# victorramirez952/tomography_3d_reconstructor

Measured on AMD Instinct MI355X. Metric: Mvoxels/s (SDF+MC) on 1024^3 ellipsoid stack; achieved HBM GB/s vs peak, higher is better.
Workload: dtype f64

## Files before the change

tomography_3d_reconstructor_amd/csrc/mesh.hip:

```cpp
#include <cstring>
#include <cstdlib>
#include "tomo_common.h"
#include <rocprim/rocprim.hpp>

__global__ __launch_bounds__(256) void vertex_finalize_kernel(float *__restrict__ vpos, int64_t nv, int shift,
                                                              const double *__restrict__ cum, int64_t ncum,
                                                              const double *__restrict__ adj, int64_t nadj, float mm_y,
                                                              float mm_x)
{
    int64_t i = (int64_t)blockIdx.x * blockDim.x + threadIdx.x;
    if (i >= nv) return;
    float *p = vpos + 3 * i;
    float z = p[0], y = p[1], x = p[2];
    if (shift) { z -= 1.0f; y -= 1.0f; x -= 1.0f; }
    if (nadj > 0) {
        if (z < 0.0f) z = 0.0f;
        else if ((double)z >= (double)(ncum - 1)) z = (float)cum[ncum - 1];
        else {
            int64_t lo = (int64_t)floorf(z);
            float frac = z - (float)lo;
            int64_t k = lo < nadj - 1 ? lo : nadj - 1;
            z = (float)(cum[lo] + (double)frac * adj[k]);
        }
    }
    p[0] = z; p[1] = y * mm_y; p[2] = x * mm_x;
}

TOMO_API int tomo_vertex_finalize(float *vpos, int64_t nv, int shift, const double *cum, int64_t ncum, const double *adj,
                                  int64_t nadj, float mm_y, float mm_x, void *stream)
{
    if (nv < 0 || (nv > 0 && !vpos) || (nadj > 0 && (!cum || !adj || ncum != nadj + 1))) return TOMO_E_ARG;
    if (nv == 0) return TOMO_OK;
    int64_t blocks = ceil_div64(nv, 256);
    if (blocks > 0x7fffffff) return TOMO_E_SIZE;
    hipLaunchKernelGGL(vertex_finalize_kernel, dim3((unsigned)blocks), dim3(256), 0, (hipStream_t)stream, vpos, nv, shift,
                       cum, ncum, adj, nadj, mm_y, mm_x);
    return tomo_status();
}

__device__ static inline u32 fkey32(float f)
{
    u32 u = __float_as_uint(f);
    return (u & 0x80000000u) ? ~u : (u | 0x80000000u);
}

__global__ __launch_bounds__(256) void uq_init_kernel(const float *__restrict__ vpos, int64_t nv, u32 *__restrict__ kx,
                                                      u32 *__restrict__ idx)
{
    int64_t i = (int64_t)blockIdx.x * blockDim.x + threadIdx.x;
    if (i >= nv) return;
    kx[i] = fkey32(vpos[3 * i + 2]);
    idx[i] = (u32)i;
}

__global__ __launch_bounds__(256) void uq_gather_kernel(const float *__restrict__ vpos, int64_t nv,
                                                        const u32 *__restrict__ idx, u64 *__restrict__ kzy)
{
    int64_t i = (int64_t)blockIdx.x * blockDim.x + threadIdx.x;
    if (i >= nv) return;
    const float *p = vpos + 3 * (int64_t)idx[i];
    kzy[i] = ((u64)fkey32(p[0]) << 32) | (u64)fkey32(p[1]);
}

__global__ __launch_bounds__(256) void uq_heads_kernel(const float *__restrict__ vpos, int64_t nv,
                                                       const u32 *__restrict__ idx, u32 *__restrict__ head)
{
    int64_t i = (int64_t)blockIdx.x * blockDim.x + threadIdx.x;
    if (i >= nv) return;
    u32 h = 1;
    if (i > 0) {
        const float *a = vpos + 3 * (int64_t)idx[i], *b = vpos + 3 * (int64_t)idx[i - 1];
        h = (a[0] != b[0] || a[1] != b[1] || a[2] != b[2]) ? 1u : 0u;
    }
    head[i] = h;
}

__global__ __launch_bounds__(256) void uq_scatter_kernel(const float *__restrict__ vpos, int64_t nv,
                                                         const u32 *__restrict__ idx, const u32 *__restrict__ head,
                                                         const u32 *__restrict__ hscan, float *__restrict__ uniq,
                                                         int32_t *__restrict__ rank, u64 *__restrict__ totals)
{
    int64_t i = (int64_t)blockIdx.x * blockDim.x + threadIdx.x;
    if (i >= nv) return;
    u32 u = hscan[i] - 1u;
    u32 src = idx[i];
    rank[src] = (int32_t)u;
    if (head[i]) {
        const float *p = vpos + 3 * (int64_t)src;
        float *q = uniq + 3 * (int64_t)u;
        q[0] = p[0]; q[1] = p[1]; q[2] = p[2];
    }
    if (i == nv - 1) totals[0] = (u64)hscan[i];
}

struct UqLayout {
    size_t kx_a, kx_b, idx_a, idx_b, idx_c, kzy_a, kzy_b, head, hscan, temp, temp_bytes, total;
};

static inline size_t align_up(size_t x, size_t a) { return (x + a - 1) / a * a; }

static UqLayout uq_layout(int64_t nv)
{
    UqLayout L;
    size_t n = (size_t)(nv > 0 ? nv : 1), off = 0;
    auto take = [&](size_t bytes) { size_t o = off; off = align_up(off + bytes, 256); return o; };
    L.kx_a = take(n * 4); L.kx_b = take(n * 4);
    L.idx_a = take(n * 4); L.idx_b = take(n * 4); L.idx_c = take(n * 4);
    L.kzy_a = take(n * 8); L.kzy_b = take(n * 8);
    L.head = take(n * 4); L.hscan = take(n * 4);
    size_t t1 = 0, t2 = 0, t3 = 0;
    (void)rocprim::radix_sort_pairs(nullptr, t1, (u32 *)nullptr, (u32 *)nullptr, (u32 *)nullptr, (u32 *)nullptr, n, 0, 32,
                              (hipStream_t)0);
    (void)rocprim::radix_sort_pairs(nullptr, t2, (u64 *)nullptr, (u64 *)nullptr, (u32 *)nullptr, (u32 *)nullptr, n, 0, 64,
                              (hipStream_t)0);
    (void)rocprim::inclusive_scan(nullptr, t3, (u32 *)nullptr, (u32 *)nullptr, n, rocprim::plus<u32>(), (hipStream_t)0);
    L.temp_bytes = t1 > t2 ? t1 : t2;
    if (t3 > L.temp_bytes) L.temp_bytes = t3;
    L.temp = take(L.temp_bytes + 256);
    L.total = off;
    return L;
}

TOMO_API int64_t tomo_mesh_unique_workspace_bytes(int64_t nv) { return (int64_t)uq_layout(nv).total; }

TOMO_API int tomo_mesh_unique(const float *vpos, int64_t nv, float *uniq, int32_t *rank, unsigned long long *totals,
                              void *workspace, int64_t workspace_bytes, void *stream)
{
    if (!vpos || !uniq || !rank || !totals || !workspace || nv <= 0) return TOMO_E_ARG;
    if (nv >= 0x7fffffffll) return TOMO_E_SIZE;
    UqLayout L = uq_layout(nv);
    if ((size_t)workspace_bytes < L.total) return TOMO_E_WORKSPACE;
    char *ws = (char *)workspace;
    u32 *kx_a = (u32 *)(ws + L.kx_a), *kx_b = (u32 *)(ws + L.kx_b);
    u32 *idx_a = (u32 *)(ws + L.idx_a), *idx_b = (u32 *)(ws + L.idx_b), *idx_c = (u32 *)(ws + L.idx_c);
    u64 *kzy_a = (u64 *)(ws + L.kzy_a), *kzy_b = (u64 *)(ws + L.kzy_b);
    u32 *head = (u32 *)(ws + L.head), *hscan = (u32 *)(ws + L.hscan);
    void *temp = ws + L.temp;
    size_t tb = L.temp_bytes;
    hipStream_t s = (hipStream_t)stream;
    unsigned blocks = (unsigned)ceil_div64(nv, 256);
    hipLaunchKernelGGL(uq_init_kernel, dim3(blocks), dim3(256), 0, s, vpos, nv, kx_a, idx_a);
    if (rocprim::radix_sort_pairs(temp, tb, kx_a, kx_b, idx_a, idx_b, (size_t)nv, 0, 32, s) != hipSuccess) return TOMO_E_LAUNCH;
    hipLaunchKernelGGL(uq_gather_kernel, dim3(blocks), dim3(256), 0, s, vpos, nv, (const u32 *)idx_b, kzy_a);
    tb = L.temp_bytes;
    if (rocprim::radix_sort_pairs(temp, tb, kzy_a, kzy_b, idx_b, idx_c, (size_t)nv, 0, 64, s) != hipSuccess) return TOMO_E_LAUNCH;
    hipLaunchKernelGGL(uq_heads_kernel, dim3(blocks), dim3(256), 0, s, vpos, nv, (const u32 *)idx_c, head);
    tb = L.temp_bytes;
    if (rocprim::inclusive_scan(temp, tb, head, hscan, (size_t)nv, rocprim::plus<u32>(), s) != hipSuccess) return TOMO_E_LAUNCH;
    hipLaunchKernelGGL(uq_scatter_kernel, dim3(blocks), dim3(256), 0, s, vpos, nv, (const u32 *)idx_c, (const u32 *)head,
                       (const u32 *)hscan, uniq, rank, (u64 *)totals);
    return tomo_status();
}

#define UQ_MAX_SLABS 65536

typedef rocprim::segmented_radix_sort_config<8, rocprim::kernel_config<512, 8>, rocprim::WarpSortConfig<32, 4, 256, 0x7fffffff, 32, 4, 256>, true>
    UqSegCfg;

struct UqOrder {
    const u32 *idx, *alt, *off;
    __device__ u32 at(u32 i) const
    {
        if (off != nullptr && i >= off[1] && i < off[3]) return alt[i];
        return idx[i];
    }
};

__device__ static inline bool rec_less(const float4 &a, const float4 &b)
{
    return a.x < b.x || (a.x == b.x && (a.y < b.y || (a.y == b.y && a.z < b.z)));
}

__global__ __launch_bounds__(256) void uq3_merge_kernel(const float4 *__restrict__ vrec, const u32 *__restrict__ off,
                                                        const u32 *__restrict__ idx, u32 *__restrict__ alt)
{
    const u32 o1 = off[1], o2 = off[2], o3 = off[3];
    const u32 na = o2 - o1, nb = o3 - o2;
    for (u32 t = blockIdx.x * blockDim.x + threadIdx.x; t < na + nb; t += gridDim.x * blockDim.x) {
        const bool inA = t < na;
        const u32 src = idx[inA ? o1 + t : o2 + (t - na)];
        const float4 k = vrec[src];
        const u32 base = inA ? o2 : o1;
        u32 lo = 0, hi = inA ? nb : na;
        while (lo < hi) {
            const u32 mid = lo + ((hi - lo) >> 1);
            const float4 m = vrec[idx[base + mid]];
            const bool less = rec_less(m, k);
            const bool equal = m.x == k.x && m.y == k.y && m.z == k.z;
            if (less || (!inA && equal)) lo = mid + 1; else hi = mid;
        }
        alt[o1 + (inA ? t : t - na) + lo] = src;
    }
}

__global__ __launch_bounds__(256) void uq3_rank_kernel(const float4 *__restrict__ vrec, int64_t cap_v, const UqOrder ord,
                                                       float *__restrict__ uniq, int32_t *__restrict__ table,
                                                       u64 *__restrict__ tot, const float z_top)
{
    const int64_t i = (int64_t)blockIdx.x * blockDim.x + threadIdx.x;
    bool viol = false;
    const u64 nv = tot[1];
    const bool live = tot[3] == 0 && i < cap_v && (u64)i < nv;
    float4 a = make_float4(0.f, 0.f, 0.f, 0.f);
    if (live) {
        u32 sa = ord.at((u32)i);
        if ((u64)sa >= nv) { sa = 0; viol = true; }
        a = vrec[sa];
    }
    float4 b;
    b.x = __shfl_up(a.x, 1, 64); b.y = __shfl_up(a.y, 1, 64); b.z = __shfl_up(a.z, 1, 64);
    if (live) {
        if ((threadIdx.x & 63) == 0 && i > 0) {
            u32 sb = ord.at((u32)i - 1u);
            if ((u64)sb >= nv) { sb = 0; viol = true; }
            b = vrec[sb];
        }
        if (i > 0) viol = viol || !rec_less(b, a);
        typedef float f3u __attribute__((ext_vector_type(3), aligned(4)));
        *(f3u *)(uniq + 3 * i) = (f3u){a.x, a.y, a.z};
        table[__float_as_uint(a.w)] = (int32_t)i;
    }
    const u64 n = (u64)__popcll(__ballot(viol));
    if ((threadIdx.x & 63) == 0 && n) atomicAdd((unsigned long long *)&tot[4], (unsigned long long)n);
    const u64 nt = (u64)__popcll(__ballot(live && a.x == z_top));
    if ((threadIdx.x & 63) == 0 && nt) atomicAdd((unsigned long long *)&tot[7], (unsigned long long)nt);
}

struct Uq3Layout { size_t keys_alt, idx_alt, idx_merge, temp, temp_bytes, total; };

static Uq3Layout uq3_layout(int64_t cap_v, int64_t nseg)
{
    Uq3Layout L;
    size_t n = (size_t)(cap_v > 0 ? cap_v : 1), off = 0;
    auto take = [&](size_t bytes) { size_t o = off; off = align_up(off + bytes, 256); return o; };
    L.keys_alt = take(n * 4); L.idx_alt = take(n * 4); L.idx_merge = take(n * 4);
    size_t t = 0;
    (void)rocprim::segmented_radix_sort_pairs<UqSegCfg>(nullptr, t, (u32 *)nullptr, (u32 *)nullptr, (u32 *)nullptr, (u32 *)nullptr,
                                                        (unsigned)n, (unsigned)(nseg > 0 ? nseg : 1), (const u32 *)nullptr,
                                                        (const u32 *)nullptr, 0, 32, (hipStream_t)0);
    L.temp_bytes = t;
    L.temp = take(t + 256);
    L.total = off;
    return L;
}

TOMO_API int64_t tomo_mc3_sort_workspace_bytes(int64_t cap_v, int64_t nseg) { return (int64_t)uq3_layout(cap_v, nseg).total; }

TOMO_API int tomo_mc3_sort_rank_top(const float *vrec, uint32_t *keys, uint32_t *idx, int64_t cap_v, int Nz, int Ny,
                                    const uint32_t *slice_tab, unsigned long long *tot, float *uniq, int32_t *table, void *workspace,
                                    int64_t workspace_bytes, float z_top, void *stream)
{
    if (!vrec || !keys || !idx || !slice_tab || !tot || !uniq || !table || !workspace || cap_v <= 0 || Nz < 1 || Ny < 1) return TOMO_E_ARG;
    if (cap_v >= 0x7fffffffll || Nz > UQ_MAX_SLABS) return TOMO_E_SIZE;
    const int64_t nseg = (int64_t)(TOMO_SORT_NB(Ny) + 1) * Nz;
    if (nseg >= 0x7fffffffll) return TOMO_E_SIZE;
    Uq3Layout L = uq3_layout(cap_v, nseg);
    if ((size_t)workspace_bytes < L.total) return TOMO_E_WORKSPACE;
    char *ws = (char *)workspace;
    u32 *keys_alt = (u32 *)(ws + L.keys_alt), *idx_alt = (u32 *)(ws + L.idx_alt), *idx_merge = (u32 *)(ws + L.idx_merge);
    const u32 *offsets = slice_tab + 2 * ((int64_t)Nz + 1);
    const u32 *merge3 = offsets + nseg + 1;
    hipStream_t s = (hipStream_t)stream;
    size_t tb = L.temp_bytes;
    if (rocprim::segmented_radix_sort_pairs<UqSegCfg>(ws + L.temp, tb, keys, keys_alt, idx, idx_alt, (unsigned)cap_v, (unsigned)nseg,
                                                      offsets, offsets + 1, 0, 32, s) != hipSuccess)
        return TOMO_E_LAUNCH;
    UqOrder order{(const u32 *)idx_alt, nullptr, nullptr};
    if (Nz >= 2) {
        hipLaunchKernelGGL(uq3_merge_kernel, dim3(256), dim3(256), 0, s, (const float4 *)vrec, merge3 - 1, (const u32 *)idx_alt, idx_merge);
        order.alt = idx_merge;
        order.off = merge3 - 1;
    }
    hipLaunchKernelGGL(uq3_rank_kernel, dim3((unsigned)ceil_div64(cap_v, 256)), dim3(256), 0, s, (const float4 *)vrec, cap_v, order,
                       uniq, table, (u64 *)tot, z_top);
    return tomo_status();
}

#define SR_THREADS 256
#define SR_E 8
#define SR_CAP 4096
#define SR_HALF 2048
#define SR_PAD(i) ((i) + ((i) >> 3))
#define SR_WORDS(cap) ((cap) + ((cap) >> 3))
#define SR_RUN (64 * SR_E)

template <int M>
__device__ static inline u32 sr_lane_xor(u32 x, const int lane)
{
    const int v = (int)x;
    if (M == 1) return (u32)__builtin_amdgcn_update_dpp(v, v, 0xB1 , 0xf, 0xf, false);
    if (M == 2) return (u32)__builtin_amdgcn_update_dpp(v, v, 0x4E , 0xf, 0xf, false);
    if (M == 8) return (u32)__builtin_amdgcn_update_dpp(v, v, 0x128 , 0xf, 0xf, false);
    if (M == 4) {
        const int up = __builtin_amdgcn_update_dpp(v, v, 0x104 , 0xf, 0xf, false);
        const int dn = __builtin_amdgcn_update_dpp(v, v, 0x114 , 0xf, 0xf, false);
        return (u32)((lane & 4) ? dn : up);
    }
    return (u32)__shfl_xor(v, M, 64);
}
template <int M>
__device__ static inline u64 sr_shfl_xor(u64 v, const int lane)
{
    return ((u64)sr_lane_xor<M>((u32)(v >> 32), lane) << 32) | sr_lane_xor<M>((u32)v, lane);
}

template <int K, int J>
__device__ static inline void sr_stage(u64 (&v)[SR_E], const int lane)
{
    if (J >= SR_E) {
        constexpr int M = J / SR_E;
        const bool keep_min = ((((lane * SR_E) & K) == 0) == ((lane & M) == 0));
#pragma unroll
        for (int r = 0; r < SR_E; r++) {
            const u64 o = sr_shfl_xor<(M > 0 ? M : 1)>(v[r], lane);
            v[r] = (keep_min == (o < v[r])) ? o : v[r];
        }
    } else {
#pragma unroll
        for (int r = 0; r < SR_E; r++) {
            if ((r & J) == 0) {
                const bool up = K < SR_E ? ((r & K) == 0) : (((lane * SR_E) & K) == 0);
                const u64 x = v[r], y = v[r | J];
                const bool sw = (y < x) == up;
                v[r] = sw ? y : x;
                v[r | J] = sw ? x : y;
            }
        }
    }
}
template <int K, int J>
struct SrLevel {
    __device__ static inline void run(u64 (&v)[SR_E], const int lane)
    {
        sr_stage<K, J>(v, lane);
        SrLevel<K, J / 2>::run(v, lane);
    }
};
template <int K>
struct SrLevel<K, 0> {
    __device__ static inline void run(u64 (&)[SR_E], const int) {}
};
template <int K>
struct SrNet {
    __device__ static inline void run(u64 (&v)[SR_E], const int lane)
    {
        SrNet<K / 2>::run(v, lane);
        SrLevel<K, K / 2>::run(v, lane);
    }
};
template <>
struct SrNet<1> {
    __device__ static inline void run(u64 (&)[SR_E], const int) {}
};
__device__ static inline void sr_wave_sort(u64 (&v)[SR_E], const int lane) { SrNet<SR_RUN>::run(v, lane); }

template <typename Make>
__device__ static u64 *sr_sort(u64 *a, u64 *b, const int n, Make make)
{
    const int tid = threadIdx.x, lane = tid & 63, wave = tid >> 6;
    for (int base = wave * SR_RUN; base < n; base += (SR_THREADS / 64) * SR_RUN) {
        const int g0 = base + lane * SR_E;
        u64 v[SR_E];
#pragma unroll
        for (int k = 0; k < SR_E; k++) v[k] = g0 + k < n ? make(g0 + k) : ~0ull;
        sr_wave_sort(v, lane);
#pragma unroll
        for (int k = 0; k < SR_E; k++) a[SR_PAD(g0) + k] = v[k];
    }
    u64 *src = a, *dst = b;
    for (int L = SR_RUN; L < n; L <<= 1) {
        __syncthreads();
        for (int g0 = tid * SR_E; g0 < n; g0 += SR_THREADS * SR_E) {
            const int pb = g0 & ~(2 * L - 1);
            const int la = n - pb < L ? n - pb : L;
            const int lb = n - pb - L < 0 ? 0 : (n - pb - L < L ? n - pb - L : L);
            const int a0 = pb, b0 = pb + L, d = g0 - pb;
            u64 out[SR_E];
            if (lb == 0 || src[SR_PAD(a0 + la - 1)] < src[SR_PAD(b0)]) {
#pragma unroll
                for (int k = 0; k < SR_E; k++) out[k] = src[SR_PAD(g0) + k];
            } else {
                int lo = d - lb > 0 ? d - lb : 0, hi = d < la ? d : la;
                while (lo < hi) {
                    const int mid = (lo + hi) >> 1;
                    if (src[SR_PAD(a0 + mid)] < src[SR_PAD(b0 + d - 1 - mid)]) lo = mid + 1; else hi = mid;
                }
                int ia = lo, ib = d - lo;
                u64 va = ia < la ? src[SR_PAD(a0 + ia)] : ~0ull, vb = ib < lb ? src[SR_PAD(b0 + ib)] : ~0ull;
#pragma unroll
                for (int k = 0; k < SR_E; k++) {
                    const bool ta = va < vb;
                    out[k] = ta ? va : vb;
                    ia += ta ? 1 : 0; ib += ta ? 0 : 1;
                    const int nx = ta ? a0 + ia : b0 + ib;
                    const bool ok = ta ? ia < la : ib < lb;
                    const u64 w = ok ? src[SR_PAD(nx)] : ~0ull;
                    va = ta ? w : va; vb = ta ? vb : w;
                }
            }
#pragma unroll
            for (int k = 0; k < SR_E; k++) dst[SR_PAD(g0) + k] = out[k];
        }
        u64 *t = src; src = dst; dst = t;
    }
    __syncthreads();
    return src;
}

__global__ __launch_bounds__(SR_THREADS) void uq3_sortrank_kernel(const float4 *__restrict__ vrec, const u32 *__restrict__ keys,
                                                                  const u32 *__restrict__ offsets, const int NB, const int Nz,
                                                                  float *__restrict__ uniq, int32_t *__restrict__ table,
                                                                  u64 *__restrict__ tot, const float z_top)
{
    constexpr int CAP = SR_HALF, EP = CAP / SR_THREADS;
    extern __shared__ __attribute__((aligned(16))) u64 s_buf[];
    u64 *const s_a = s_buf, *const s_b = s_buf + SR_WORDS(CAP);
    float4 *const s_rows = (float4 *)s_buf;
    u32 *const s_red = (u32 *)s_b;
    const int tid = threadIdx.x, lane = tid & 63, wave = tid >> 6;
    const int seg = (blockIdx.x & 1) ? (int)gridDim.x - 1 - (int)(blockIdx.x >> 1) : (int)(blockIdx.x >> 1);
    u32 o0 = offsets[seg];
    int n = (int)(offsets[seg + 1] - o0);
    const u64 nv = tot[1];
    bool uni = false;
    if (Nz >= 2 && seg >= NB && seg <= 2 * NB) {
        const u32 o1 = offsets[NB], o2 = offsets[NB + 1], o3 = offsets[2 * NB + 1];
        if (o2 > o1 && o3 > o2) {
            u32 kmax = 0;
            for (u32 i = o1 + tid; i < o2; i += SR_THREADS) kmax = max(kmax, keys[i]);
#pragma unroll
            for (int d = 32; d > 0; d >>= 1) kmax = max(kmax, (u32)__shfl_xor((int)kmax, d, 64));
            if (lane == 0) s_red[wave] = kmax;
            __syncthreads();
            kmax = max(max(s_red[0], s_red[1]), max(s_red[2], s_red[3]));
            if (kmax >= fkey32(vrec[o2].x)) {
                if (seg == NB) { uni = true; o0 = o1; n = (int)(o3 - o1); }
                else n = 0;
            }
            __syncthreads();
        }
    }
    constexpr int UCAP = CAP / 2 / SR_RUN * SR_RUN;
    if (n > (uni ? UCAP : SR_CAP)) {
        if (tid == 0) atomicOr((unsigned long long *)&tot[3], 8ull);
        return;
    }
    if (n == 0) return;
    if (n > CAP) {
        const int nB = n - CAP;
        const u64 *sa = sr_sort(s_a, s_b, CAP, [=](int i) { return ((u64)keys[o0 + i] << 32) | (u32)i; });
        u64 ra[EP], rb[EP];
#pragma unroll
        for (int e = 0; e < EP; e++) ra[e] = sa[SR_PAD(tid + SR_THREADS * e)];
        __syncthreads();
        const u64 *sb = sr_sort(s_a, s_b, nB, [=](int i) { return ((u64)keys[o0 + CAP + i] << 32) | (u32)(CAP + i); });
#pragma unroll
        for (int e = 0; e < EP; e++) rb[e] = sb[SR_PAD(min(tid + SR_THREADS * e, nB - 1))];
        __syncthreads();
        u64 *const M = s_buf;
#define SR_MP(i) ((i) + ((i) >> 4))
#pragma unroll
        for (int e = 0; e < EP; e++) {
            const int i = tid + SR_THREADS * e;
            M[SR_MP(i)] = ra[e];
            if (i < nB) M[SR_MP(CAP + i)] = rb[e];
        }
        float4 *const s_tail = (float4 *)(s_buf + SR_MP(SR_CAP) + 2);
        __syncthreads();
        constexpr int EO = SR_CAP / SR_THREADS;
        const int g0 = tid * EO < n ? tid * EO : n;
        int lo = g0 - nB > 0 ? g0 - nB : 0, hi = g0 < CAP ? g0 : CAP;
        while (lo < hi) {
            const int mid = (lo + hi) >> 1;
            if (M[SR_MP(mid)] < M[SR_MP(CAP + g0 - 1 - mid)]) lo = mid + 1; else hi = mid;
        }
        int ia = lo, ib = g0 - lo;
        u64 va = ia < CAP ? M[SR_MP(ia)] : ~0ull, vb = ib < nB ? M[SR_MP(CAP + ib)] : ~0ull;
        float4 r[EO];
#pragma unroll
        for (int k = 0; k < EO; k++) {
            const bool ta = va < vb;
            const u64 w = ta ? va : vb;
            ia += ta ? 1 : 0; ib += ta ? 0 : 1;
            const bool ok = ta ? ia < CAP : ib < nB;
            const u64 nw = ok ? M[SR_MP(ta ? ia : CAP + ib)] : ~0ull;
            va = ta ? nw : va; vb = ta ? vb : nw;
            r[k] = vrec[o0 + (w == ~0ull ? 0u : (u32)w)];
        }
#pragma unroll
        for (int k = 0; k < EO; k++) asm volatile("" : "+v"(r[k].x), "+v"(r[k].y), "+v"(r[k].z), "+v"(r[k].w));
        float4 below;
        below.x = __shfl_up(r[EO - 1].x, 1, 64); below.y = __shfl_up(r[EO - 1].y, 1, 64); below.z = __shfl_up(r[EO - 1].z, 1, 64);
        if (lane == 63) s_tail[wave] = r[EO - 1];
        __syncthreads();
        if (lane == 0 && wave > 0) below = s_tail[wave - 1];
        u32 nviol = 0, ntop = 0;
        float4 prev = below;
#pragma unroll
        for (int k = 0; k < EO; k++) {
            const int i = tid * EO + k;
            if (i < n && (u64)(o0 + i) < nv) {
                if (i > 0 && !rec_less(prev, r[k])) nviol++;
                typedef float f3u __attribute__((ext_vector_type(3), aligned(4)));
                *(f3u *)(uniq + 3 * (int64_t)(o0 + i)) = (f3u){r[k].x, r[k].y, r[k].z};
                table[__float_as_uint(r[k].w)] = (int32_t)(o0 + i);
                if (r[k].x == z_top) ntop++;
            }
            prev = r[k];
        }
        nviol = wave_sum(nviol); ntop = wave_sum(ntop);
        if (lane == 0 && nviol) atomicAdd((unsigned long long *)&tot[4], (unsigned long long)nviol);
        if (lane == 0 && ntop) atomicAdd((unsigned long long *)&tot[7], (unsigned long long)ntop);
        return;
    }
    const u64 *sorted;
    const u32 *first = nullptr;
    if (!uni) {
        sorted = sr_sort(s_a, s_b, n, [=](int i) { return ((u64)keys[o0 + i] << 32) | (u32)i; });
    } else {
        u64 *const h0 = s_a, *const h1 = s_a + SR_WORDS(UCAP);
        const u64 *p1 = sr_sort(h0, h1, n, [=](int i) { return ((u64)fkey32(vrec[o0 + i].z) << 32) | (u32)i; });
        u32 *ord = (u32 *)s_b;
        for (int i = tid; i < n; i += SR_THREADS) ord[i] = (u32)p1[SR_PAD(i)];
        __syncthreads();
        sorted = sr_sort(h0, h1, n, [=](int i) { return ((u64)fkey32(vrec[o0 + ord[i]].y) << 32) | (u32)i; });
        first = ord;
    }
    u32 p[EP];
#pragma unroll
    for (int e = 0; e < EP; e++) {
        const int i = tid + SR_THREADS * e, ii = i < n ? i : n - 1;
        const u32 q = (u32)sorted[SR_PAD(ii)];
        p[e] = first ? first[q] : q;
    }
    __syncthreads();
    float4 r[EP];
#pragma unroll
    for (int e = 0; e < EP; e++) r[e] = vrec[o0 + p[e]];
#pragma unroll
    for (int e = 0; e < EP; e++)
        asm volatile("" : "+v"(r[e].x), "+v"(r[e].y), "+v"(r[e].z), "+v"(r[e].w));
#pragma unroll
    for (int e = 0; e < EP; e++) if (tid + SR_THREADS * e < n) s_rows[tid + SR_THREADS * e] = r[e];
    __syncthreads();
    u32 nviol = 0, ntop = 0;
#pragma unroll
    for (int e = 0; e < EP; e++) {
        const int i = tid + SR_THREADS * e;
        if (i < n && (u64)(o0 + i) < nv) {
            const float4 a = s_rows[i];
            if (i > 0 && !rec_less(s_rows[i - 1], a)) nviol++;
            typedef float f3u __attribute__((ext_vector_type(3), aligned(4)));
            *(f3u *)(uniq + 3 * (int64_t)(o0 + i)) = (f3u){a.x, a.y, a.z};
            table[__float_as_uint(a.w)] = (int32_t)(o0 + i);
            if (a.x == z_top) ntop++;
        }
    }
    nviol = wave_sum(nviol); ntop = wave_sum(ntop);
    if (lane == 0 && nviol) atomicAdd((unsigned long long *)&tot[4], (unsigned long long)nviol);
    if (lane == 0 && ntop) atomicAdd((unsigned long long *)&tot[7], (unsigned long long)ntop);
}

__global__ __launch_bounds__(256) void uq3_seams_kernel(const float *__restrict__ uniq, const u32 *__restrict__ offsets, const int nseg,
                                                        u64 *__restrict__ tot)
{
    const int s = 1 + blockIdx.x * blockDim.x + threadIdx.x;
    bool bad = false;
    if (s < nseg && tot[3] == 0) {
        const u32 q0 = offsets[s];
        if (q0 != 0 && (u64)q0 < tot[1] && offsets[s + 1] != q0) {
            const float *r = uniq + 3 * (int64_t)(q0 - 1);
            bad = !(r[0] < r[3] || (r[0] == r[3] && (r[1] < r[4] || (r[1] == r[4] && r[2] < r[5]))));
        }
    }
    const u64 nbad = (u64)__popcll(__ballot(bad));
    if ((threadIdx.x & 63) == 0 && nbad) atomicAdd((unsigned long long *)&tot[4], (unsigned long long)nbad);
}

TOMO_API int tomo_mc3_sort_rank_fused(const float *vrec, const uint32_t *keys, int64_t cap_v, int Nz, int Ny, uint32_t *slice_tab,
                                      unsigned long long *tot, float *uniq, int32_t *table, float z_top, void *stream)
{
    if (!vrec || !keys || !slice_tab || !tot || !uniq || !table || cap_v <= 0 || Nz < 1 || Ny < 1) return TOMO_E_ARG;
    if (cap_v >= 0x7fffffffll || Nz > UQ_MAX_SLABS) return TOMO_E_SIZE;
    const int NB = TOMO_SORT_NB(Ny);
    const int64_t nseg = (int64_t)(NB + 1) * Nz;
    if (nseg >= 0x7fffffffll) return TOMO_E_SIZE;
    const u32 *offsets = slice_tab + 2 * ((int64_t)Nz + 1);
    hipStream_t s = (hipStream_t)stream;
    const size_t lds = 2 * SR_WORDS(SR_HALF) * sizeof(u64);
    hipLaunchKernelGGL(uq3_sortrank_kernel, dim3((unsigned)nseg), dim3(SR_THREADS), lds, s, (const float4 *)vrec, (const u32 *)keys,
                       offsets, NB, Nz, uniq, table, (u64 *)tot, z_top);
    hipLaunchKernelGGL(uq3_seams_kernel, dim3((unsigned)ceil_div64(nseg, 256)), dim3(256), 0, s, (const float *)uniq, offsets, (int)nseg,
                       (u64 *)tot);
    return tomo_status();
}

__global__ __launch_bounds__(256) void rows_lookup_kernel(const float *__restrict__ uniq, int64_t nu,
                                                          const float *__restrict__ query, int64_t nq,
                                                          int32_t *__restrict__ out, u64 *__restrict__ missing)
{
    int64_t i = (int64_t)blockIdx.x * blockDim.x + threadIdx.x;
    if (i >= nq) return;
    const float qz = query[3 * i], qy = query[3 * i + 1], qx = query[3 * i + 2];
    int64_t lo = 0, hi = nu;
    while (lo < hi) {
        const int64_t mid = lo + ((hi - lo) >> 1);
        const float *m = uniq + 3 * mid;
        const bool less = m[0] < qz || (m[0] == qz && (m[1] < qy || (m[1] == qy && m[2] < qx)));
        if (less) lo = mid + 1; else hi = mid;
    }
    const bool found = lo < nu && uniq[3 * lo] == qz && uniq[3 * lo + 1] == qy && uniq[3 * lo + 2] == qx;
    out[i] = found ? (int32_t)lo : -1;
    if (!found) atomicAdd(missing, 1ull);
}

TOMO_API int tomo_mesh_lookup(const float *uniq, int64_t nu, const float *query, int64_t nq, int32_t *out,
                              unsigned long long *missing, void *stream)
{
    if (nq < 0 || nu < 0 || (nq > 0 && (!query || !out || !missing)) || (nu > 0 && !uniq)) return TOMO_E_ARG;
    if (nq == 0) return TOMO_OK;
    if (nu >= 0x7fffffffll) return TOMO_E_SIZE;
    hipLaunchKernelGGL(rows_lookup_kernel, dim3((unsigned)ceil_div64(nq, 256)), dim3(256), 0, (hipStream_t)stream, uniq, nu,
                       query, nq, out, (u64 *)missing);
    return tomo_status();
}

__device__ static inline bool slab_counts_ok(const u64 *tot, int64_t cap_v)
{
    return tot[3] == 0 && tot[1] <= (u64)cap_v && tot[7] <= tot[1];
}

__global__ __launch_bounds__(256) void slab_top_rows_kernel(const float *__restrict__ uniq, const u64 *__restrict__ tot,
                                                            int64_t cap_v, int64_t cap, float *__restrict__ msg)
{
    const int64_t i = (int64_t)blockIdx.x * blockDim.x + threadIdx.x;
    const bool ok = slab_counts_ok(tot, cap_v);
    const u64 nv = ok ? tot[1] : 0, nt = ok ? tot[7] : 0;
    if (i == 0) {
        msg[0] = __uint_as_float((u32)(nt < 0xffffffffull ? nt : 0xffffffffull));
        msg[1] = msg[2] = 0.f;
    }
    if (i >= cap) return;
    float z = 0.f, y = 0.f, x = 0.f;
    if ((u64)i < nt) {
        const float *src = uniq + 3 * (nv - nt + (u64)i);
        z = src[0]; y = src[1]; x = src[2];
    }
    msg[3 + 3 * i] = z; msg[4 + 3 * i] = y; msg[5 + 3 * i] = x;
}

__global__ __launch_bounds__(256) void slab_lookup_kernel(const float *__restrict__ uniq, const u64 *__restrict__ tot,
                                                          int64_t cap_v, const float *__restrict__ msg, int64_t cap,
                                                          int32_t *__restrict__ out, u64 *__restrict__ missing)
{
    const int64_t i = (int64_t)blockIdx.x * blockDim.x + threadIdx.x;
    if (i >= cap) return;
    const int64_t nu = slab_counts_ok(tot, cap_v) ? (int64_t)tot[1] : 0;
    const int64_t nq = (int64_t)__float_as_uint(msg[0]);
    if (i >= nq) { out[i] = -1; return; }
    const float qz = msg[3 + 3 * i], qy = msg[4 + 3 * i], qx = msg[5 + 3 * i];
    int64_t lo = 0, hi = nu;
    while (lo < hi) {
        const int64_t mid = lo + ((hi - lo) >> 1);
        const float *m = uniq + 3 * mid;
        const bool less = m[0] < qz || (m[0] == qz && (m[1] < qy || (m[1] == qy && m[2] < qx)));
        if (less) lo = mid + 1; else hi = mid;
    }
    const bool found = lo < nu && uniq[3 * lo] == qz && uniq[3 * lo + 1] == qy && uniq[3 * lo + 2] == qx;
    out[i] = found ? (int32_t)lo : -1;
    if (!found) atomicAdd((unsigned long long *)missing, 1ull);
}

__global__ void slab_summary_kernel(const u64 *__restrict__ tot, int64_t cap_v, const float *__restrict__ msg_in,
                                    u64 *__restrict__ missing, int64_t cap_top, int64_t caller_flags,
                                    int64_t *__restrict__ out)
{
    if (blockIdx.x | threadIdx.x) return;
    int64_t flags = caller_flags ? 8 : 0;
    if (tot[3] != 0 || tot[1] > (u64)cap_v || tot[7] > tot[1]) flags |= 1;
    if (tot[4] != 0) flags |= 2;
    if (tot[7] > (u64)cap_top) flags |= 4;
    const int64_t from_prev = msg_in ? (int64_t)__float_as_uint(msg_in[0]) : 0;
    out[0] = (flags & 1) ? 0 : (int64_t)(tot[1] - tot[7]);
    out[1] = missing ? (int64_t)*missing : 0;
    if (missing) *missing = 0ull;
    out[2] = flags;
    out[3] = (int64_t)tot[1];
    out[4] = (int64_t)tot[7];
    out[5] = from_prev;
    out[6] = (int64_t)tot[0];
    out[7] = (int64_t)tot[2];
}

__global__ __launch_bounds__(256) void slab_lookup_summary_kernel(const float *__restrict__ uniq, const u64 *__restrict__ tot,
                                                                  int64_t cap_v, const float *__restrict__ msg, int64_t cap,
                                                                  int32_t *__restrict__ out, int64_t cap_top, int64_t caller_flags,
                                                                  u64 *__restrict__ scratch, int64_t *__restrict__ summary)
{
    __shared__ int s_last;
    bool missed = false;
    if (msg != nullptr) {
        const int64_t i = (int64_t)blockIdx.x * blockDim.x + threadIdx.x;
        const int64_t nu = slab_counts_ok(tot, cap_v) ? (int64_t)tot[1] : 0;
        const int64_t nq = (int64_t)__float_as_uint(msg[0]);
        if (i < cap) {
            if (i >= nq) out[i] = -1;
            else {
                const float qz = msg[3 + 3 * i], qy = msg[4 + 3 * i], qx = msg[5 + 3 * i];
                int64_t lo = 0, hi = nu;
                while (lo < hi) {
                    const int64_t mid = lo + ((hi - lo) >> 1);
                    const float *m = uniq + 3 * mid;
                    const bool less = m[0] < qz || (m[0] == qz && (m[1] < qy || (m[1] == qy && m[2] < qx)));
                    if (less) lo = mid + 1; else hi = mid;
                }
                const bool found = lo < nu && uniq[3 * lo] == qz && uniq[3 * lo + 1] == qy && uniq[3 * lo + 2] == qx;
                out[i] = found ? (int32_t)lo : -1;
                missed = !found;
            }
        }
    }
    const u64 nm = (u64)__popcll(__ballot(missed));
    if ((threadIdx.x & 63) == 0 && nm) atomicAdd((unsigned long long *)&scratch[1], (unsigned long long)nm);
    __threadfence();
    __syncthreads();
    if (threadIdx.x == 0) s_last = atomicAdd((unsigned long long *)&scratch[0], 1ull) == (unsigned long long)gridDim.x - 1ull;
    __syncthreads();
    if (!s_last || threadIdx.x != 0) return;
    __threadfence();
    const u64 misses = atomicExch((unsigned long long *)&scratch[1], 0ull);
    scratch[0] = 0ull;
    int64_t flags = caller_flags ? 8 : 0;
    if (tot[3] != 0 || tot[1] > (u64)cap_v || tot[7] > tot[1]) flags |= 1;
    if (tot[4] != 0) flags |= 2;
    if (tot[7] > (u64)cap_top) flags |= 4;
    summary[0] = (flags & 1) ? 0 : (int64_t)(tot[1] - tot[7]);
    summary[1] = (int64_t)misses;
    summary[2] = flags;
    summary[3] = (int64_t)tot[1];
    summary[4] = (int64_t)tot[7];
    summary[5] = msg ? (int64_t)__float_as_uint(msg[0]) : 0;
    summary[6] = (int64_t)tot[0];
    summary[7] = (int64_t)tot[2];
}

TOMO_API int tomo_slab_lookup_summary(const float *uniq, const unsigned long long *tot, int64_t cap_v, const float *msg, int64_t cap,
                                      int32_t *out, int64_t cap_top, int64_t caller_flags, unsigned long long *scratch, int64_t *summary,
                                      void *stream)
{
    if (!uniq || !tot || !summary || !scratch || cap_v < 1 || cap_top < 0 || (msg && (!out || cap < 1))) return TOMO_E_ARG;
    const int64_t blocks = msg ? ceil_div64(cap, 256) : 1;
    if (blocks > 0x7fffffff) return TOMO_E_SIZE;
    hipLaunchKernelGGL(slab_lookup_summary_kernel, dim3((unsigned)blocks), dim3(256), 0, (hipStream_t)stream, uniq, (const u64 *)tot,
                       cap_v, msg, cap, out, cap_top, caller_flags, (u64 *)scratch, summary);
    return tomo_status();
}

TOMO_API int tomo_slab_top_rows(const float *uniq, const unsigned long long *tot, int64_t cap_v, int64_t cap, float *msg, void *stream)
{
    if (!uniq || !tot || !msg || cap < 1 || cap_v < 1) return TOMO_E_ARG;
    hipLaunchKernelGGL(slab_top_rows_kernel, dim3((unsigned)ceil_div64(cap, 256)), dim3(256), 0, (hipStream_t)stream, uniq,
                       (const u64 *)tot, cap_v, cap, msg);
    return tomo_status();
}

TOMO_API int tomo_slab_lookup(const float *uniq, const unsigned long long *tot, int64_t cap_v, const float *msg, int64_t cap,
                              int32_t *out, unsigned long long *missing, void *stream)
{
    if (!uniq || !tot || !msg || !out || !missing || cap < 1 || cap_v < 1) return TOMO_E_ARG;
    hipLaunchKernelGGL(slab_lookup_kernel, dim3((unsigned)ceil_div64(cap, 256)), dim3(256), 0, (hipStream_t)stream, uniq,
                       (const u64 *)tot, cap_v, msg, cap, out, (u64 *)missing);
    return tomo_status();
}

TOMO_API int tomo_slab_summary(const unsigned long long *tot, int64_t cap_v, const float *msg_in, unsigned long long *missing,
                               int64_t cap_top, int64_t caller_flags, int64_t *out, void *stream)
{
    if (!tot || !out || cap_v < 1 || cap_top < 0) return TOMO_E_ARG;
    hipLaunchKernelGGL(slab_summary_kernel, dim3(1), dim3(64), 0, (hipStream_t)stream, (const u64 *)tot, cap_v, msg_in,
                       (u64 *)missing, cap_top, caller_flags, out);
    return tomo_status();
}

__global__ __launch_bounds__(256) void volume_area_kernel(const float *__restrict__ v, const int64_t *__restrict__ faces,
                                                          int64_t nf, double *__restrict__ out)
{
    double vol = 0.0, area = 0.0;
    for (int64_t f = (int64_t)blockIdx.x * blockDim.x + threadIdx.x; f < nf; f += (int64_t)gridDim.x * blockDim.x) {
        const float *a = v + 3 * faces[3 * f], *b = v + 3 * faces[3 * f + 1], *c = v + 3 * faces[3 * f + 2];
        float cx = b[1] * c[2] - b[2] * c[1], cy = b[2] * c[0] - b[0] * c[2], cz = b[0] * c[1] - b[1] * c[0];
        float d = a[0] * cx + a[1] * cy + a[2] * cz;
        vol += (double)d / 6.0;
        float ux = b[0] - a[0], uy = b[1] - a[1], uz = b[2] - a[2];
        float wx = c[0] - a[0], wy = c[1] - a[1], wz = c[2] - a[2];
        float nx = uy * wz - uz * wy, ny = uz * wx - ux * wz, nz = ux * wy - uy * wx;
        float nrm = sqrtf(nx * nx + ny * ny + nz * nz);
        area += (double)(0.5f * nrm);
    }
#pragma unroll
    for (int d = 32; d > 0; d >>= 1) { vol += __shfl_xor(vol, d, 64); area += __shfl_xor(area, d, 64); }
    if ((threadIdx.x & 63) == 0) { atomicAdd(&out[0], vol); atomicAdd(&out[1], area); }
}

TOMO_API int tomo_mesh_volume_area(const float *verts, const int64_t *faces, int64_t nf, double *out, void *stream)
{
    if (!verts || !faces || !out || nf < 0) return TOMO_E_ARG;
    if (nf == 0) return TOMO_OK;
    int64_t blocks = ceil_div64(nf, 256);
    if (blocks > 1024) blocks = 1024;
    hipLaunchKernelGGL(volume_area_kernel, dim3((unsigned)blocks), dim3(256), 0, (hipStream_t)stream, verts, faces, nf, out);
    return tomo_status();
}
```

Before: 659,300.

## Add 32-bit packed-key sort path and optional local-rank sort in segment sort-rank

Result: no change. 662,700 (median of 5 runs) (+0.5%).

```diff
diff --git a/tomography_3d_reconstructor_amd/csrc/mesh.hip b/tomography_3d_reconstructor_amd/csrc/mesh.hip
--- a/tomography_3d_reconstructor_amd/csrc/mesh.hip
+++ b/tomography_3d_reconstructor_amd/csrc/mesh.hip
@@ -283,6 +283,21 @@
 #define SR_PAD(i) ((i) + ((i) >> 3))
 #define SR_WORDS(cap) ((cap) + ((cap) >> 3))
 #define SR_RUN (64 * SR_E)
+#define SR_RANK_MAX 128
+#define SR_P_RANK 1
+#define SR_P_NET32 2
+
+template <typename W, int PB> struct SrWord;
+template <int PB> struct SrWord<u64, PB> {
+    __device__ static inline bool fits(u32, u32) { return true; }
+    __device__ static inline u64 make(u32 key, u32, u32 pos) { return ((u64)key << 32) | pos; }
+    __device__ static inline u32 pos(u64 w) { return (u32)w; }
+};
+template <int PB> struct SrWord<u32, PB> {
+    __device__ static inline bool fits(u32 kmin, u32 kmax) { return kmax - kmin < (1u << (32 - PB)) - 1u; }
+    __device__ static inline u32 make(u32 key, u32 kmin, u32 pos) { return ((key - kmin) << PB) | pos; }
+    __device__ static inline u32 pos(u32 w) { return w & ((1u << PB) - 1u); }
+};
 
 template <int M>
 __device__ static inline u32 sr_lane_xor(u32 x, const int lane)
@@ -303,16 +318,18 @@
 {
     return ((u64)sr_lane_xor<M>((u32)(v >> 32), lane) << 32) | sr_lane_xor<M>((u32)v, lane);
 }
-
-template <int K, int J>
-__device__ static inline void sr_stage(u64 (&v)[SR_E], const int lane)
+template <int M>
+__device__ static inline u32 sr_shfl_xor(u32 v, const int lane) { return sr_lane_xor<M>(v, lane); }
+
+template <int K, int J, typename W>
+__device__ static inline void sr_stage(W (&v)[SR_E], const int lane)
 {
     if (J >= SR_E) {
         constexpr int M = J / SR_E;
         const bool keep_min = ((((lane * SR_E) & K) == 0) == ((lane & M) == 0));
 #pragma unroll
         for (int r = 0; r < SR_E; r++) {
-            const u64 o = sr_shfl_xor<(M > 0 ? M : 1)>(v[r], lane);
+            const W o = sr_shfl_xor<(M > 0 ? M : 1)>(v[r], lane);
             v[r] = (keep_min == (o < v[r])) ? o : v[r];
         }
     } else {
@@ -320,7 +337,7 @@
         for (int r = 0; r < SR_E; r++) {
             if ((r & J) == 0) {
                 const bool up = K < SR_E ? ((r & K) == 0) : (((lane * SR_E) & K) == 0);
-                const u64 x = v[r], y = v[r | J];
+                const W x = v[r], y = v[r | J];
                 const bool sw = (y < x) == up;
                 v[r] = sw ? y : x;
                 v[r | J] = sw ? x : y;
@@ -330,7 +347,8 @@
 }
 template <int K, int J>
 struct SrLevel {
-    __device__ static inline void run(u64 (&v)[SR_E], const int lane)
+    template <typename W>
+    __device__ static inline void run(W (&v)[SR_E], const int lane)
     {
         sr_stage<K, J>(v, lane);
         SrLevel<K, J / 2>::run(v, lane);
@@ -338,11 +356,13 @@
 };
 template <int K>
 struct SrLevel<K, 0> {
-    __device__ static inline void run(u64 (&)[SR_E], const int) {}
+    template <typename W>
+    __device__ static inline void run(W (&)[SR_E], const int) {}
 };
 template <int K>
 struct SrNet {
-    __device__ static inline void run(u64 (&v)[SR_E], const int lane)
+    template <typename W>
+    __device__ static inline void run(W (&v)[SR_E], const int lane)
     {
         SrNet<K / 2>::run(v, lane);
         SrLevel<K, K / 2>::run(v, lane);
@@ -350,24 +370,27 @@
 };
 template <>
 struct SrNet<1> {
-    __device__ static inline void run(u64 (&)[SR_E], const int) {}
+    template <typename W>
+    __device__ static inline void run(W (&)[SR_E], const int) {}
 };
-__device__ static inline void sr_wave_sort(u64 (&v)[SR_E], const int lane) { SrNet<SR_RUN>::run(v, lane); }
-
-template <typename Make>
-__device__ static u64 *sr_sort(u64 *a, u64 *b, const int n, Make make)
-{
+template <typename W>
+__device__ static inline void sr_wave_sort(W (&v)[SR_E], const int lane) { SrNet<SR_RUN>::run(v, lane); }
+
+template <typename W, typename Make>
+__device__ static W *sr_sort(W *a, W *b, const int n, Make make)
+{
+    constexpr W ones = (W) ~(W)0;
     const int tid = threadIdx.x, lane = tid & 63, wave = tid >> 6;
     for (int base = wave * SR_RUN; base < n; base += (SR_THREADS / 64) * SR_RUN) {
         const int g0 = base + lane * SR_E;
-        u64 v[SR_E];
-#pragma unroll
-        for (int k = 0; k < SR_E; k++) v[k] = g0 + k < n ? make(g0 + k) : ~0ull;
+        W v[SR_E];
+#pragma unroll
+        for (int k = 0; k < SR_E; k++) v[k] = g0 + k < n ? make(g0 + k) : ones;
         sr_wave_sort(v, lane);
 #pragma unroll
         for (int k = 0; k < SR_E; k++) a[SR_PAD(g0) + k] = v[k];
     }
-    u64 *src = a, *dst = b;
+    W *src = a, *dst = b;
     for (int L = SR_RUN; L < n; L <<= 1) {
         __syncthreads();
         for (int g0 = tid * SR_E; g0 < n; g0 += SR_THREADS * SR_E) {
@@ -375,7 +398,7 @@
             const int la = n - pb < L ? n - pb : L;
             const int lb = n - pb - L < 0 ? 0 : (n - pb - L < L ? n - pb - L : L);
             const int a0 = pb, b0 = pb + L, d = g0 - pb;
-            u64 out[SR_E];
+            W out[SR_E];
             if (lb == 0 || src[SR_PAD(a0 + la - 1)] < src[SR_PAD(b0)]) {
 #pragma unroll
                 for (int k = 0; k < SR_E; k++) out[k] = src[SR_PAD(g0) + k];
@@ -386,7 +409,7 @@
                     if (src[SR_PAD(a0 + mid)] < src[SR_PAD(b0 + d - 1 - mid)]) lo = mid + 1; else hi = mid;
                 }
                 int ia = lo, ib = d - lo;
-                u64 va = ia < la ? src[SR_PAD(a0 + ia)] : ~0ull, vb = ib < lb ? src[SR_PAD(b0 + ib)] : ~0ull;
+                W va = ia < la ? src[SR_PAD(a0 + ia)] : ones, vb = ib < lb ? src[SR_PAD(b0 + ib)] : ones;
 #pragma unroll
                 for (int k = 0; k < SR_E; k++) {
                     const bool ta = va < vb;
@@ -394,29 +417,215 @@
                     ia += ta ? 1 : 0; ib += ta ? 0 : 1;
                     const int nx = ta ? a0 + ia : b0 + ib;
                     const bool ok = ta ? ia < la : ib < lb;
-                    const u64 w = ok ? src[SR_PAD(nx)] : ~0ull;
+                    const W w = ok ? src[SR_PAD(nx)] : ones;
                     va = ta ? w : va; vb = ta ? vb : w;
                 }
             }
 #pragma unroll
             for (int k = 0; k < SR_E; k++) dst[SR_PAD(g0) + k] = out[k];
         }
-        u64 *t = src; src = dst; dst = t;
+        W *t = src; src = dst; dst = t;
     }
     __syncthreads();
     return src;
+}
+
+__device__ static inline void sr_block_minmax(u32 &kmin, u32 &kmax, u32 *x)
+{
+    const int lane = threadIdx.x & 63, wave = threadIdx.x >> 6;
+    kmin = wave_min32(kmin); kmax = wave_max32(kmax);
+    if (lane == 0) { x[wave] = kmin; x[4 + wave] = kmax; }
+    __syncthreads();
+    kmin = min(min(x[0], x[1]), min(x[2], x[3]));
+    kmax = max(max(x[4], x[5]), max(x[6], x[7]));
+    __syncthreads();
+}
+
+__device__ static inline u32 sr_scan_max_up(u32 v, const int lane)
+{
+#pragma unroll
+    for (int d = 1; d < 64; d <<= 1) {
+        const u32 o = (u32)__shfl_up((int)v, d, 64);
+        if (lane >= d) v = max(v, o);
+    }
+    return v;
+}
+__device__ static inline u32 sr_scan_min_down(u32 v, const int lane)
+{
+#pragma unroll
+    for (int d = 1; d < 64; d <<= 1) {
+        const u32 o = (u32)__shfl_down((int)v, d, 64);
+        if (lane + d < 64) v = min(v, o);
+    }
+    return v;
+}
+
+__device__ static bool sr_rank(const u32 *key, u32 *perm, u32 *x, const int n)
+{
+    const int tid = threadIdx.x, lane = tid & 63, wave = tid >> 6, g0 = tid * SR_E;
+    u32 k[SR_E], pm[SR_E], sm[SR_E];
+#pragma unroll
+    for (int j = 0; j < SR_E; j++) k[j] = g0 + j < n ? key[SR_PAD(g0) + j] : ~0u;
+    pm[0] = k[0];
+#pragma unroll
+    for (int j = 1; j < SR_E; j++) pm[j] = max(pm[j - 1], k[j]);
+    sm[SR_E - 1] = k[SR_E - 1];
+#pragma unroll
+    for (int j = SR_E - 2; j >= 0; j--) sm[j] = min(sm[j + 1], k[j]);
+    const u32 ip = sr_scan_max_up(pm[SR_E - 1], lane), is = sr_scan_min_down(sm[0], lane);
+    u32 ep = (u32)__shfl_up((int)ip, 1, 64), es = (u32)__shfl_down((int)is, 1, 64);
+    if (lane == 0) ep = 0u;
+    if (lane == 63) es = ~0u;
+    if (lane == 63) x[wave] = ip;
+    if (lane == 0) x[4 + wave] = is;
+    __syncthreads();
+#pragma unroll
+    for (int w = 0; w < SR_THREADS / 64; w++) {
+        if (w < wave) ep = max(ep, x[w]);
+        if (w > wave) es = min(es, x[4 + w]);
+    }
+    bool c[SR_E];
+    c[0] = ep <= min(es, sm[0]);
+#pragma unroll
+    for (int j = 1; j < SR_E; j++) c[j] = max(ep, pm[j - 1]) <= min(es, sm[j]);
+    u32 last = 0u, first = SR_HALF;
+#pragma unroll
+    for (int j = 0; j < SR_E; j++) last = c[j] ? (u32)(g0 + j) : last;
+#pragma unroll
+    for (int j = SR_E - 1; j >= 0; j--) first = c[j] ? (u32)(g0 + j) : first;
+    const u32 il = sr_scan_max_up(last, lane), ifi = sr_scan_min_down(first, lane);
+    u32 el = (u32)__shfl_up((int)il, 1, 64), ef = (u32)__shfl_down((int)ifi, 1, 64);
+    if (lane == 0) el = 0u;
+    if (lane == 63) ef = SR_HALF;
+    if (lane == 63) x[8 + wave] = il;
+    if (lane == 0) x[12 + wave] = ifi;
+    __syncthreads();
+#pragma unroll
+    for (int w = 0; w < SR_THREADS / 64; w++) {
+        if (w < wave) el = max(el, x[8 + w]);
+        if (w > wave) ef = min(ef, x[12 + w]);
+    }
+    u32 st[SR_E], en[SR_E];
+    st[0] = c[0] ? (u32)g0 : el;
+#pragma unroll
+    for (int j = 1; j < SR_E; j++) st[j] = c[j] ? (u32)(g0 + j) : st[j - 1];
+    en[SR_E - 1] = ef;
+#pragma unroll
+    for (int j = SR_E - 2; j >= 0; j--) en[j] = c[j + 1] ? (u32)(g0 + j + 1) : en[j + 1];
+    u32 mine = 0u;
+#pragma unroll
+    for (int j = 0; j < SR_E; j++) mine = g0 + j < n ? max(mine, en[j] - st[j]) : mine;
+    const u32 wl = wave_max32(mine);
+    if (lane == 0) x[16 + wave] = wl;
+    __syncthreads();
+    if (max(max(x[16], x[17]), max(x[18], x[19])) > SR_RANK_MAX) return false;
+    const u32 lo = st[0], hi = g0 < n ? min(en[SR_E - 1], (u32)n) : lo;
+    u64 w[SR_E];
+    u32 cnt[SR_E];
+#pragma unroll
+    for (int j = 0; j < SR_E; j++) { w[j] = ((u64)k[j] << 32) | (u32)(g0 + j); cnt[j] = 0u; }
+    for (u32 q = lo; q < hi; q++) {
+        const u64 wq = ((u64)key[SR_PAD(q)] << 32) | q;
+#pragma unroll
+        for (int j = 0; j < SR_E; j++) cnt[j] += wq < w[j] ? 1u : 0u;
+    }
+#pragma unroll
+    for (int j = 0; j < SR_E; j++)
+        if (g0 + j < n) perm[lo + cnt[j]] = (u32)(g0 + j);
+    __syncthreads();
+    return true;
+}
+
+#define SR_MP(i) ((i) + ((i) >> 4))
+template <typename W>
+__device__ static __forceinline__ void sr_long_segment(u64 *s_buf, const float4 *__restrict__ vrec, const u32 *__restrict__ keys,
+                                                       const u32 o0, const int n, const u32 kmin, const u64 nv,
+                                                       float *__restrict__ uniq, int32_t *__restrict__ table, u64 *__restrict__ tot,
+                                                       const float z_top)
+{
+    typedef SrWord<W, 12> Word;
+    constexpr W ones = (W) ~(W)0;
+    constexpr int CAP = SR_HALF, EP = CAP / SR_THREADS;
+    const int tid = threadIdx.x, lane = tid & 63, wave = tid >> 6;
+    W *const s_a = (W *)s_buf, *const s_b = (W *)s_buf + SR_WORDS(CAP);
+    const int nB = n - CAP;
+    const W *sa = sr_sort<W>(s_a, s_b, CAP, [=](int i) { return Word::make(keys[o0 + i], kmin, (u32)i); });
+    W ra[EP], rb[EP];
+#pragma unroll
+    for (int e = 0; e < EP; e++) ra[e] = sa[SR_PAD(tid + SR_THREADS * e)];
+    __syncthreads();
+    const W *sb = sr_sort<W>(s_a, s_b, nB, [=](int i) { return Word::make(keys[o0 + CAP + i], kmin, (u32)(CAP + i)); });
+#pragma unroll
+    for (int e = 0; e < EP; e++) rb[e] = sb[SR_PAD(min(tid + SR_THREADS * e, nB - 1))];
+    __syncthreads();
+    W *const M = (W *)s_buf;
+#pragma unroll
+    for (int e = 0; e < EP; e++) {
+        const int i = tid + SR_THREADS * e;
+        M[SR_MP(i)] = ra[e];
+        if (i < nB) M[SR_MP(CAP + i)] = rb[e];
+    }
+    float4 *const s_tail = (float4 *)(s_buf + SR_MP(SR_CAP) + 2);
+    __syncthreads();
+    constexpr int EO = SR_CAP / SR_THREADS;
+    const int g0 = tid * EO < n ? tid * EO : n;
+    int lo = g0 - nB > 0 ? g0 - nB : 0, hi = g0 < CAP ? g0 : CAP;
+    while (lo < hi) {
+        const int mid = (lo + hi) >> 1;
+        if (M[SR_MP(mid)] < M[SR_MP(CAP + g0 - 1 - mid)]) lo = mid + 1; else hi = mid;
+    }
+    int ia = lo, ib = g0 - lo;
+    W va = ia < CAP ? M[SR_MP(ia)] : ones, vb = ib < nB ? M[SR_MP(CAP + ib)] : ones;
+    float4 r[EO];
+#pragma unroll
+    for (int k = 0; k < EO; k++) {
+        const bool ta = va < vb;
+        const W w = ta ? va : vb;
+        ia += ta ? 1 : 0; ib += ta ? 0 : 1;
+        const bool ok = ta ? ia < CAP : ib < nB;
+        const W nw = ok ? M[SR_MP(ta ? ia : CAP + ib)] : ones;
+        va = ta ? nw : va; vb = ta ? vb : nw;
+        r[k] = vrec[o0 + (w == ones ? 0u : Word::pos(w))];
+    }
+#pragma unroll
+    for (int k = 0; k < EO; k++) asm volatile("" : "+v"(r[k].x), "+v"(r[k].y), "+v"(r[k].z), "+v"(r[k].w));
+    float4 below;
+    below.x = __shfl_up(r[EO - 1].x, 1, 64); below.y = __shfl_up(r[EO - 1].y, 1, 64); below.z = __shfl_up(r[EO - 1].z, 1, 64);
+    if (lane == 63) s_tail[wave] = r[EO - 1];
+    __syncthreads();
+    if (lane == 0 && wave > 0) below = s_tail[wave - 1];
+    u32 nviol = 0, ntop = 0;
+    float4 prev = below;
+#pragma unroll
+    for (int k = 0; k < EO; k++) {
+        const int i = tid * EO + k;
+        if (i < n && (u64)(o0 + i) < nv) {
+            if (i > 0 && !rec_less(prev, r[k])) nviol++;
+            typedef float f3u __attribute__((ext_vector_type(3), aligned(4)));
+            *(f3u *)(uniq + 3 * (int64_t)(o0 + i)) = (f3u){r[k].x, r[k].y, r[k].z};
+            table[__float_as_uint(r[k].w)] = (int32_t)(o0 + i);
+            if (r[k].x == z_top) ntop++;
+        }
+        prev = r[k];
+    }
+    nviol = wave_sum(nviol); ntop = wave_sum(ntop);
+    if (lane == 0 && nviol) atomicAdd((unsigned long long *)&tot[4], (unsigned long long)nviol);
+    if (lane == 0 && ntop) atomicAdd((unsigned long long *)&tot[7], (unsigned long long)ntop);
 }
 
 __global__ __launch_bounds__(SR_THREADS) void uq3_sortrank_kernel(const float4 *__restrict__ vrec, const u32 *__restrict__ keys,
                                                                   const u32 *__restrict__ offsets, const int NB, const int Nz,
                                                                   float *__restrict__ uniq, int32_t *__restrict__ table,
-                                                                  u64 *__restrict__ tot, const float z_top)
+                                                                  u64 *__restrict__ tot, const float z_top, const int paths)
 {
     constexpr int CAP = SR_HALF, EP = CAP / SR_THREADS;
     extern __shared__ __attribute__((aligned(16))) u64 s_buf[];
     u64 *const s_a = s_buf, *const s_b = s_buf + SR_WORDS(CAP);
     float4 *const s_rows = (float4 *)s_buf;
     u32 *const s_red = (u32 *)s_b;
+    u32 *const s_a32 = (u32 *)s_buf, *const s_b32 = s_a32 + SR_WORDS(CAP);
+    u32 *const s_perm = s_a32 + 2 * SR_WORDS(CAP), *const s_x = s_perm + CAP;
+    u32 *const s_key = s_a32 + 3 * SR_WORDS(CAP);
     const int tid = threadIdx.x, lane = tid & 63, wave = tid >> 6;
     const int seg = (blockIdx.x & 1) ? (int)gridDim.x - 1 - (int)(blockIdx.x >> 1) : (int)(blockIdx.x >> 1);
     u32 o0 = offsets[seg];
@@ -445,92 +654,57 @@
         if (tid == 0) atomicOr((unsigned long long *)&tot[3], 8ull);
         return;
     }
-    if (n == 0) return;
+    if (n <= 0) return;
     if (n > CAP) {
-        const int nB = n - CAP;
-        const u64 *sa = sr_sort(s_a, s_b, CAP, [=](int i) { return ((u64)keys[o0 + i] << 32) | (u32)i; });
-        u64 ra[EP], rb[EP];
-#pragma unroll
-        for (int e = 0; e < EP; e++) ra[e] = sa[SR_PAD(tid + SR_THREADS * e)];
-        __syncthreads();
-        const u64 *sb = sr_sort(s_a, s_b, nB, [=](int i) { return ((u64)keys[o0 + CAP + i] << 32) | (u32)(CAP + i); });
-#pragma unroll
-        for (int e = 0; e < EP; e++) rb[e] = sb[SR_PAD(min(tid + SR_THREADS * e, nB - 1))];
-        __syncthreads();
-        u64 *const M = s_buf;
-#define SR_MP(i) ((i) + ((i) >> 4))
-#pragma unroll
-        for (int e = 0; e < EP; e++) {
-            const int i = tid + SR_THREADS * e;
-            M[SR_MP(i)] = ra[e];
-            if (i < nB) M[SR_MP(CAP + i)] = rb[e];
-        }
-        float4 *const s_tail = (float4 *)(s_buf + SR_MP(SR_CAP) + 2);
-        __syncthreads();
-        constexpr int EO = SR_CAP / SR_THREADS;
-        const int g0 = tid * EO < n ? tid * EO : n;
-        int lo = g0 - nB > 0 ? g0 - nB : 0, hi = g0 < CAP ? g0 : CAP;
-        while (lo < hi) {
-            const int mid = (lo + hi) >> 1;
-            if (M[SR_MP(mid)] < M[SR_MP(CAP + g0 - 1 - mid)]) lo = mid + 1; else hi = mid;
-        }
-        int ia = lo, ib = g0 - lo;
-        u64 va = ia < CAP ? M[SR_MP(ia)] : ~0ull, vb = ib < nB ? M[SR_MP(CAP + ib)] : ~0ull;
-        float4 r[EO];
-#pragma unroll
-        for (int k = 0; k < EO; k++) {
-            const bool ta = va < vb;
-            const u64 w = ta ? va : vb;
-            ia += ta ? 1 : 0; ib += ta ? 0 : 1;
-            const bool ok = ta ? ia < CAP : ib < nB;
-            const u64 nw = ok ? M[SR_MP(ta ? ia : CAP + ib)] : ~0ull;
-            va = ta ? nw : va; vb = ta ? vb : nw;
-            r[k] = vrec[o0 + (w == ~0ull ? 0u : (u32)w)];
-        }
-#pragma unroll
-        for (int k = 0; k < EO; k++) asm volatile("" : "+v"(r[k].x), "+v"(r[k].y), "+v"(r[k].z), "+v"(r[k].w));
-        float4 below;
-        below.x = __shfl_up(r[EO - 1].x, 1, 64); below.y = __shfl_up(r[EO - 1].y, 1, 64); below.z = __shfl_up(r[EO - 1].z, 1, 64);
-        if (lane == 63) s_tail[wave] = r[EO - 1];
-        __syncthreads();
-        if (lane == 0 && wave > 0) below = s_tail[wave - 1];
-        u32 nviol = 0, ntop = 0;
-        float4 prev = below;
-#pragma unroll
-        for (int k = 0; k < EO; k++) {
-            const int i = tid * EO + k;
-            if (i < n && (u64)(o0 + i) < nv) {
-                if (i > 0 && !rec_less(prev, r[k])) nviol++;
-                typedef float f3u __attribute__((ext_vector_type(3), aligned(4)));
-                *(f3u *)(uniq + 3 * (int64_t)(o0 + i)) = (f3u){r[k].x, r[k].y, r[k].z};
-                table[__float_as_uint(r[k].w)] = (int32_t)(o0 + i);
-                if (r[k].x == z_top) ntop++;
+        u32 kmin = ~0u, kmax = 0u;
+        if (paths & SR_P_NET32) {
+            for (int i = tid; i < n; i += SR_THREADS) {
+                const u32 k = keys[o0 + i];
+                kmin = min(kmin, k); kmax = max(kmax, k);
             }
-            prev = r[k];
-        }
-        nviol = wave_sum(nviol); ntop = wave_sum(ntop);
-        if (lane == 0 && nviol) atomicAdd((unsigned long long *)&tot[4], (unsigned long long)nviol);
-        if (lane == 0 && ntop) atomicAdd((unsigned long long *)&tot[7], (unsigned long long)ntop);
+            sr_block_minmax(kmin, kmax, s_a32);
+        }
+        if ((paths & SR_P_NET32) && SrWord<u32, 12>::fits(kmin, kmax))
+            sr_long_segment<u32>(s_buf, vrec, keys, o0, n, kmin, nv, uniq, table, tot, z_top);
+        else
+            sr_long_segment<u64>(s_buf, vrec, keys, o0, n, 0u, nv, uniq, table, tot, z_top);
         return;
     }
-    const u64 *sorted;
+    const u64 *sorted = nullptr;
+    const u32 *sorted32 = nullptr;
     const u32 *first = nullptr;
     if (!uni) {
-        sorted = sr_sort(s_a, s_b, n, [=](int i) { return ((u64)keys[o0 + i] << 32) | (u32)i; });
+        u32 kmin = ~0u, kmax = 0u;
+        for (int i = tid; i < n; i += SR_THREADS) {
+            const u32 k = keys[o0 + i];
+            s_key[SR_PAD(i)] = k;
+            kmin = min(kmin, k); kmax = max(kmax, k);
+        }
+        __syncthreads();
+        if (!((paths & SR_P_RANK) && sr_rank(s_key, s_perm, s_x, n))) {
+            typedef SrWord<u32, 11> Word;
+            bool narrow = false;
+            if (paths & SR_P_NET32) {
+                sr_block_minmax(kmin, kmax, s_x + 24);
+                narrow = Word::fits(kmin, kmax);
+            }
+            if (narrow) sorted32 = sr_sort<u32>(s_a32, s_b32, n, [=](int i) { return Word::make(s_key[SR_PAD(i)], kmin, (u32)i); });
+            else sorted = sr_sort<u64>(s_a, s_b, n, [=](int i) { return ((u64)s_key[SR_PAD(i)] << 32) | (u32)i; });
+        }
     } else {
         u64 *const h0 = s_a, *const h1 = s_a + SR_WORDS(UCAP);
-        const u64 *p1 = sr_sort(h0, h1, n, [=](int i) { return ((u64)fkey32(vrec[o0 + i].z) << 32) | (u32)i; });
+        const u64 *p1 = sr_sort<u64>(h0, h1, n, [=](int i) { return ((u64)fkey32(vrec[o0 + i].z) << 32) | (u32)i; });
         u32 *ord = (u32 *)s_b;
         for (int i = tid; i < n; i += SR_THREADS) ord[i] = (u32)p1[SR_PAD(i)];
         __syncthreads();
-        sorted = sr_sort(h0, h1, n, [=](int i) { return ((u64)fkey32(vrec[o0 + ord[i]].y) << 32) | (u32)i; });
+        sorted = sr_sort<u64>(h0, h1, n, [=](int i) { return ((u64)fkey32(vrec[o0 + ord[i]].y) << 32) | (u32)i; });
         first = ord;
     }
     u32 p[EP];
 #pragma unroll
     for (int e = 0; e < EP; e++) {
         const int i = tid + SR_THREADS * e, ii = i < n ? i : n - 1;
-        const u32 q = (u32)sorted[SR_PAD(ii)];
+        const u32 q = sorted ? (u32)sorted[SR_PAD(ii)] : sorted32 ? SrWord<u32, 11>::pos(sorted32[SR_PAD(ii)]) : s_perm[ii];
         p[e] = first ? first[q] : q;
     }
     __syncthreads();
@@ -586,10 +760,17 @@
     const int64_t nseg = (int64_t)(NB + 1) * Nz;
     if (nseg >= 0x7fffffffll) return TOMO_E_SIZE;
     const u32 *offsets = slice_tab + 2 * ((int64_t)Nz + 1);
+    int paths = SR_P_NET32;
+    if (const char *e = getenv("TOMO_SORT_PATHS")) {
+        if (!strcmp(e, "net64")) paths = 0;
+        else if (!strcmp(e, "rank")) paths = SR_P_RANK;
+        else if (!strcmp(e, "all")) paths = SR_P_RANK | SR_P_NET32;
+        else if (strcmp(e, "net32") && e[0]) return TOMO_E_ARG;
+    }
     hipStream_t s = (hipStream_t)stream;
     const size_t lds = 2 * SR_WORDS(SR_HALF) * sizeof(u64);
     hipLaunchKernelGGL(uq3_sortrank_kernel, dim3((unsigned)nseg), dim3(SR_THREADS), lds, s, (const float4 *)vrec, (const u32 *)keys,
-                       offsets, NB, Nz, uniq, table, (u64 *)tot, z_top);
+                       offsets, NB, Nz, uniq, table, (u64 *)tot, z_top, paths);
     hipLaunchKernelGGL(uq3_seams_kernel, dim3((unsigned)ceil_div64(nseg, 256)), dim3(256), 0, s, (const float *)uniq, offsets, (int)nseg,
                        (u64 *)tot);
     return tomo_status();
```
